# Plachtaa/FAcodec

Measured on AMD Instinct MI355X. Metric: 24kHz audio sec encoded+decoded per wall-sec, higher is better.
Workload: dtype f32; 1 GPU; configs[1]: batch=32/GPU x 2 s @ 24 kHz, forward encoder->FVQ(6 codebooks)->decoder, FAcodec configs/config.yml model (137.7 M params), weights formula-generated, weight-norm re-materialised every step; clips_per_gpu=32, samples_per_clip=48000, parallelism=dp1 (independent clips, no collective)

## Files before the change

facodec_amd/csrc/conv1d_bsplit.hip:

```cpp
#include "conv1d_mfma.h"
#include <type_traits>
#include "inflight_regs.h"
#include "prep_batch.h"

namespace fac {

typedef __bf16 bf16x8 __attribute__((ext_vector_type(8)));

constexpr int BS_CO = 64;
constexpr int BS_NSW = 4;
constexpr int BS_NSW_WIDE = 4;
constexpr int BS_XU = 3;
static int conv_device_cus() {
  static int cus[16] = {0};
  int dev = 0, v = 0;
  if (hipGetDevice(&dev) != hipSuccess || dev < 0 || dev >= 16) return 0;
  if (cus[dev] == 0 && hipDeviceGetAttribute(&v, hipDeviceAttributeMultiprocessorCount, dev) == hipSuccess) cus[dev] = v;
  return cus[dev];
}
constexpr int BS_WIDE_MIN = 64;
__host__ __device__ constexpr int bs_group(int C_in) { return C_in >= BS_WIDE_MIN ? 2 : 1; }

__device__ __forceinline__ void split3(float x, __bf16& h, __bf16& m, __bf16& l) {
  h = (__bf16)x;
  const float r1 = x - (float)h;
  m = (__bf16)r1;
  l = (__bf16)(r1 - (float)m);
}

__host__ __device__ constexpr int bs_slots(int K, int G) { return (G * K + 1) & ~1; }

__device__ __forceinline__ void pack_conv_split_body(const float* __restrict__ v, const float* __restrict__ scale,
                                                     bf16x8* __restrict__ out, int C_out, int C_in, int K, int G, int H, int n_st,
                                                     long long n, int vb, int vg) {
  for (long long idx = (long long)vb * 256 + threadIdx.x; idx < n; idx += (long long)vg * 256) {
    const int co = (int)(idx % BS_CO);
    long long r = idx / BS_CO;
    const int hs = (int)(r % H);
    r /= H;
    const int s = (int)(r % n_st);
    const int ct = (int)(r / n_st);
    const int g = hs % G, k = hs / G;
    const int cog = ct * BS_CO + co;
    const float sc = (scale != nullptr && cog < C_out) ? scale[cog] : 1.0f;
    bf16x8 h, m, l;
#pragma unroll
    for (int i = 0; i < 8; ++i) {
      const int ci = (s * G + g) * 8 + i;
      float w = 0.f;
      if (cog < C_out && ci < C_in && k < K) {
        w = v[((long long)cog * C_in + ci) * K + k];
        if (scale != nullptr) w = __fmul_rn(w, sc);
      }
      __bf16 a, b2, c;
      split3(w, a, b2, c);
      h[i] = a; m[i] = b2; l[i] = c;
    }
    const long long base = ((long long)ct * n_st + s) * 3;
    out[((base + 0) * H + hs) * BS_CO + co] = h;
    out[((base + 1) * H + hs) * BS_CO + co] = m;
    out[((base + 2) * H + hs) * BS_CO + co] = l;
  }
}

__global__ __launch_bounds__(256) void pack_conv_split_kernel(const float* __restrict__ v, const float* __restrict__ scale,
                                                              bf16x8* __restrict__ out, int C_out, int C_in, int K, int G, int H,
                                                              int n_st, long long n) {
  pack_conv_split_body(v, scale, out, C_out, C_in, K, G, H, n_st, n, blockIdx.x, gridDim.x);
}

__global__ __launch_bounds__(256) void bsplit_batch_kernel(const PrepJob* __restrict__ jobs, const int* __restrict__ first, int njobs) {
  const int j = prep_find_job(first, njobs, blockIdx.x);
  const PrepJob& J = jobs[j];
  pack_conv_split_body(static_cast<const float*>(J.a), static_cast<const float*>(J.b), static_cast<bf16x8*>(J.out), J.i[0], J.i[1],
                       J.i[2], J.i[3], J.i[4], J.i[5], J.n, blockIdx.x - first[j], J.nblocks);
}

int prep_launch_bsplit(const PrepJob* jobs, const int* first, int njobs, int total, hipStream_t s) {
  hipLaunchKernelGGL(bsplit_batch_kernel, dim3(total), dim3(256), 0, s, jobs, first, njobs);
  return check_launch("bsplit_batch");
}

template <int KT, int G, int NMW, int NSW>
__global__ __launch_bounds__((NMW + NSW) * 64, (NMW + NSW) / 4) void conv1d_bsplit_kernel(ConvArgs a) {
  constexpr int MB = 2, NB = 2;
  constexpr int BS_TT = 64 * NMW;
  constexpr int H = bs_slots(KT, G);
  constexpr int W_STAGE = 3 * H * BS_CO * 16;
  extern __shared__ __attribute__((aligned(16))) unsigned char sm[];
  const int tid = threadIdx.x;
  const int lane = tid & 63;
  const int wave = __builtin_amdgcn_readfirstlane(tid >> 6);
  const int XW = a.XW;
  const int X_STAGE = 48 * G * XW;
  const int STG = W_STAGE + X_STAGE;
  unsigned char* Wbuf = sm;
  unsigned char* Xbuf = sm + W_STAGE;
  const int n_chunks = (a.C_in + 8 * G - 1) / (8 * G);
  const int dil = a.dil;

  const int n_tiles = a.n_tiles;
  typedef const __attribute__((address_space(4))) ConvArgs* KArgP;
  const KArgP kargs = (KArgP)__builtin_amdgcn_kernarg_segment_ptr();
  auto fresh_args = [&]() {
    KArgP q = kargs;
    asm volatile("" : "+s"(q));
    return q;
  };
  auto decode = [&](KArgP ka, int v, int& t0_, int& co0_, int& b_) {
    const int q8 = n_tiles >> 3, r8 = n_tiles & 7;
    const int xcd = v & 7, within = v >> 3;
    const int id = (xcd < r8 ? xcd * (q8 + 1) : r8 * (q8 + 1) + (xcd - r8) * q8) + within;
    const int nt = ka->n_t_tiles;
    const int tt = id % nt;
    const int rest = id / nt;
    const int nb = ka->B;
    b_ = rest % nb;
    co0_ = (rest / nb) * BS_CO;
    t0_ = tt * BS_TT;
  };
  const bool overlap = a.persist != 0;
  unsigned char* epi_base = sm + (overlap ? STG : 0);
  auto walk = [&](auto role) {
  constexpr int ROLE = decltype(role)::value;
  constexpr bool STAGING = ROLE != 0;
  bool first = true;
  unsigned cboff[BS_XU] = {}, nboff[BS_XU] = {};
  unsigned long long cmask[BS_XU] = {}, nmask[BS_XU] = {};
  const float *cxg = nullptr, *nxg = nullptr;
  const unsigned char *cws = nullptr, *nws = nullptr;
  for (int vb = blockIdx.x; vb < n_tiles; vb += gridDim.x) {
  int t0, co0, b;
  decode(fresh_args(), vb, t0, co0, b);
  const bool has_nt = overlap && vb + (int)gridDim.x < n_tiles;

  if constexpr (STAGING) {
    const int lw = wave - NMW;
    __builtin_amdgcn_s_setprio(FAC_PRIO_STAGE);
    const float* xg = a.x + (long long)b * a.x_bs;
    const int xcs = (int)a.x_cs;
    const unsigned char* wsrc = reinterpret_cast<const unsigned char*>(a.w) + (long long)(co0 / BS_CO) * n_chunks * W_STAGE;
    const int n_blk = (XW + 63) >> 6;
    int u_g[BS_XU], u_c[BS_XU], u_idx[BS_XU];
#pragma unroll
    for (int j = 0; j < BS_XU; ++j) {
      const int u = lw + NSW * j;
      u_g[j] = u % G;
      const int c = (u / G) * 64 + lane;
      u_c[j] = (u < G * n_blk && c < XW) ? c : -1;
      const int tin = t0 - a.pad_left + c;
      int idx;
      if (a.pad_mode == FAC_PAD_REFLECT) idx = reflect_index(tin, a.T_in, a.T_ext);
      else idx = (tin >= 0 && tin < a.T_in) ? tin : -1;
      u_idx[j] = u_c[j] >= 0 ? idx : -1;
    }
    constexpr int NBLK = W_STAGE / 1024;
    constexpr int ND = (NBLK + NSW - 1) / NSW;
    constexpr int NX = BS_XU * 8;
    static_assert(W_STAGE % 1024 == 0 && ND + NX <= 63 && NX == 24, "vmcnt is a 6-bit counter; FAC_XREGS24_* list 24 registers per set");
    auto stage_w = [&](int chunk, int buf) {
      constexpr int N16 = W_STAGE / 16;
      const unsigned char* src = wsrc + (long long)chunk * W_STAGE;
      unsigned char* dst = Wbuf + buf * STG;
      for (int i = lw; i * 64 < N16; i += NSW) {
        const int q = i * 64 + lane;
        if (q < N16)
          __builtin_amdgcn_global_load_lds((glb_void_t*)(src + (long long)q * 16), (lds_void_t*)(dst + i * 1024), 16, 0, 0);
      }
    };
    auto write_x = [&](int buf, const float (&xr)[BS_XU][8]) {
      unsigned char* xd = Xbuf + buf * STG;
#pragma unroll
      for (int j = 0; j < BS_XU; ++j) {
        if (u_c[j] < 0) continue;
        bf16x8 h, m, l;
#pragma unroll
        for (int i = 0; i < 8; ++i) {
          __bf16 p0, p1, p2;
          split3(xr[j][i], p0, p1, p2);
          h[i] = p0; m[i] = p1; l[i] = p2;
        }
        *reinterpret_cast<bf16x8*>(xd + ((0 * G + u_g[j]) * XW + u_c[j]) * 16) = h;
        *reinterpret_cast<bf16x8*>(xd + ((1 * G + u_g[j]) * XW + u_c[j]) * 16) = m;
        *reinterpret_cast<bf16x8*>(xd + ((2 * G + u_g[j]) * XW + u_c[j]) * 16) = l;
      }
    };
    if constexpr (ROLE == 2) {
      typedef float wv4 __attribute__((ext_vector_type(4)));
      const unsigned char* xp = a.x_p8 + (long long)b * (a.C_in / 8) * a.T_in * 16;
      const long long grp_bytes = (long long)a.T_in * 16;
      unsigned u_poff[BS_XU];
      bool any_pad = false;
#pragma unroll
      for (int j = 0; j < BS_XU; ++j) {
        u_poff[j] = (unsigned)(u_idx[j] >= 0 ? u_idx[j] : 0) * 16u;
        any_pad = any_pad || __builtin_amdgcn_ballot_w64(u_c[j] >= 0 && u_idx[j] < 0) != 0;
      }
      for (int c = -1; c < n_chunks; ++c) {
        if (c + 1 < n_chunks) {
          const int buf = (c + 1) & 1;
          wv4 wv[ND], xv[BS_XU][3];
          const unsigned char* src = wsrc + (long long)(c + 1) * W_STAGE;
#pragma unroll
          for (int j = 0; j < ND; ++j) {
            const int bi = min(lw + NSW * j, NBLK - 1);
            wv[j] = *reinterpret_cast<const wv4*>(src + bi * 1024 + lane * 16);
          }
#pragma unroll
          for (int j = 0; j < BS_XU; ++j) {
            const unsigned char* grp = xp + (long long)((c + 1) * G + u_g[j]) * grp_bytes;
#pragma unroll
            for (int pl = 0; pl < 3; ++pl) xv[j][pl] = *reinterpret_cast<const wv4*>(grp + pl * a.x_p8_ps + u_poff[j]);
          }
          unsigned char* xd = Xbuf + buf * STG;
#pragma unroll
          for (int j = 0; j < BS_XU; ++j) {
            if (u_c[j] < 0) continue;
#pragma unroll
            for (int pl = 0; pl < 3; ++pl) {
              wv4 v = xv[j][pl];
              if (any_pad && u_idx[j] < 0) v = wv4{0.f, 0.f, 0.f, 0.f};
              *reinterpret_cast<wv4*>(xd + ((pl * G + u_g[j]) * XW + u_c[j]) * 16) = v;
            }
          }
          unsigned char* dst = Wbuf + buf * STG;
#pragma unroll
          for (int j = 0; j < ND; ++j) {
            const int bi = min(lw + NSW * j, NBLK - 1);
            *reinterpret_cast<wv4*>(dst + bi * 1024 + lane * 16) = wv[j];
          }
        }
        __syncthreads();
      }
    } else if constexpr (G == 2) {
#define BS_LD(n, R)                                                                                                          \
  asm volatile("global_load_dword v" #R ", %0, %1" : : "v"(u_boff[(n) / 8]), "s"(grp[(n) / 8] + (long long)((n) % 8) * xcs) : "memory", "v" #R);
#define BS_RD(n, R) asm volatile("v_cndmask_b32_e64 %0, 0, v" #R ", %1" : "=v"(xr[(n) / 8][(n) % 8]) : "s"(u_mask[(n) / 8]) : "memory");
      auto tile_params = [&](int t0_, int b_, int co0_, unsigned (&boff)[BS_XU], unsigned long long (&mask)[BS_XU], const float*& xgp,
                             const unsigned char*& wsp) {
        const KArgP ka = fresh_args();
        const int pad_left = ka->pad_left, pad_mode = ka->pad_mode, T_in = ka->T_in, T_ext = ka->T_ext;
#pragma unroll
        for (int j = 0; j < BS_XU; ++j) {
          const int tin = t0_ - pad_left + u_c[j];
          int idx;
          if (pad_mode == FAC_PAD_REFLECT) idx = reflect_index(tin, T_in, T_ext);
          else idx = (tin >= 0 && tin < T_in) ? tin : -1;
          if (u_c[j] < 0) idx = -1;
          boff[j] = (unsigned)(idx >= 0 ? idx : 0) * 4u;
          mask[j] = __builtin_amdgcn_ballot_w64(idx >= 0);
        }
        xgp = ka->x + (long long)b_ * ka->x_bs;
        wsp = reinterpret_cast<const unsigned char*>(ka->w) + (long long)(co0_ / BS_CO) * n_chunks * W_STAGE;
      };
      if (first) tile_params(t0, b, co0, cboff, cmask, cxg, cws);
      if (has_nt) {
        int nt0, nco0, nb;
        decode(fresh_args(), vb + (int)gridDim.x, nt0, nco0, nb);
        tile_params(nt0, nb, nco0, nboff, nmask, nxg, nws);
      }
      auto load_a = [&](const float* xgp, const unsigned (&u_boff)[BS_XU], int chunk) {
        const float* grp[BS_XU];
#pragma unroll
        for (int j = 0; j < BS_XU; ++j) grp[j] = xgp + (long long)((chunk * G + u_g[j]) * 8) * xcs;
        FAC_XREGS24_A(BS_LD)
      };
      auto load_b = [&](const float* xgp, const unsigned (&u_boff)[BS_XU], int chunk) {
        const float* grp[BS_XU];
#pragma unroll
        for (int j = 0; j < BS_XU; ++j) grp[j] = xgp + (long long)((chunk * G + u_g[j]) * 8) * xcs;
        FAC_XREGS24_B(BS_LD)
      };
      auto take_a = [&](float (&xr)[BS_XU][8], const unsigned long long (&u_mask)[BS_XU]) { FAC_XREGS24_A(BS_RD) };
      auto take_b = [&](float (&xr)[BS_XU][8], const unsigned long long (&u_mask)[BS_XU]) { FAC_XREGS24_B(BS_RD) };
      typedef float wv4 __attribute__((ext_vector_type(4)));
      const int wblk0 = min(lw * ND, NBLK - ND);
      const unsigned lane16 = (unsigned)lane * 16u;
      for (int base = first ? -2 : 0; base < n_chunks; base += 2) {
#pragma unroll
        for (int i = 0; i < 2; ++i) {
          const int c = base + i;
          if (c >= n_chunks) break;
          const bool nx1 = c + 1 >= n_chunks, nx2 = c + 2 >= n_chunks;
          const bool has_next = c + 1 >= 0 && (!nx1 || has_nt), has_next2 = !nx2 || has_nt;
          float xr[BS_XU][8];
          wv4 wv[ND];
          if (has_next) {
            const unsigned char* src = (nx1 ? nws : cws) + (long long)(nx1 ? c + 1 - n_chunks : c + 1) * W_STAGE + wblk0 * 1024;
#pragma unroll
            for (int j = 0; j < ND; ++j)
              asm volatile("global_load_dwordx4 %0, %1, %2" : "=v"(wv[j]) : "v"(lane16), "s"(src + j * 1024) : "memory");
            asm volatile("s_waitcnt vmcnt(%0)" : : "n"(ND) : "memory");
            unsigned long long u_mask[BS_XU];
#pragma unroll
            for (int j = 0; j < BS_XU; ++j) u_mask[j] = nx1 ? nmask[j] : cmask[j];
            if (i == 0) take_b(xr, u_mask); else take_a(xr, u_mask);
          }
          if (has_next2) {
            unsigned u_boff[BS_XU];
#pragma unroll
            for (int j = 0; j < BS_XU; ++j) u_boff[j] = nx2 ? nboff[j] : cboff[j];
            const float* xgp = nx2 ? nxg : cxg;
            const int chunk = nx2 ? c + 2 - n_chunks : c + 2;
            if (i == 0) load_a(xgp, u_boff, chunk); else load_b(xgp, u_boff, chunk);
          }
          if (has_next) {
            write_x(1 - i, xr);
            if (has_next2) asm volatile("s_waitcnt vmcnt(%0)" : : "n"(NX) : "memory");
            else asm volatile("s_waitcnt vmcnt(0)" ::: "memory");
            unsigned char* dst = Wbuf + (1 - i) * STG + wblk0 * 1024 + lane16;
#pragma unroll
            for (int j = 0; j < ND; ++j) {
              asm volatile("" : "+v"(wv[j]) : : "memory");
              *reinterpret_cast<wv4*>(dst + j * 1024) = wv[j];
            }
          }
          if (c >= -1) {
            asm volatile("s_waitcnt lgkmcnt(0)" ::: "memory");
            __builtin_amdgcn_s_barrier();
            asm volatile("" ::: "memory");
          }
        }
      }
      if (has_nt) {
#pragma unroll
        for (int j = 0; j < BS_XU; ++j) {
          cboff[j] = nboff[j];
          cmask[j] = nmask[j];
        }
        cxg = nxg;
        cws = nws;
      }
#undef BS_LD
#undef BS_RD
    } else {
      int u_off[BS_XU];
#pragma unroll
      for (int j = 0; j < BS_XU; ++j) u_off[j] = u_idx[j] >= 0 ? u_idx[j] : 0;
      auto load_x = [&](int chunk, float (&xr)[BS_XU][8]) {
#pragma unroll
        for (int j = 0; j < BS_XU; ++j) {
          const float* grp = xg + (long long)((chunk * G + u_g[j]) * 8) * xcs;
#pragma unroll
          for (int i = 0; i < 8; ++i) {
            const float v = (grp + (long long)i * xcs)[u_off[j]];
            xr[j][i] = u_idx[j] >= 0 ? v : 0.f;
          }
        }
      };
      float xa[BS_XU][8], xb[BS_XU][8];
      load_x(0, xa);
      stage_w(0, 0);
      if (n_chunks > 1) load_x(1, xb);
      write_x(0, xa);
      __syncthreads();
      for (int chunk = 0; chunk < n_chunks; chunk += 2) {
        if (chunk + 1 < n_chunks) {
          stage_w(chunk + 1, 1);
          if (chunk + 2 < n_chunks) load_x(chunk + 2, xa);
          write_x(1, xb);
        }
        __syncthreads();
        if (chunk + 1 >= n_chunks) break;
        if (chunk + 2 < n_chunks) {
          stage_w(chunk + 2, 0);
          if (chunk + 3 < n_chunks) load_x(chunk + 3, xb);
          write_x(0, xa);
        }
        __syncthreads();
      }
    }
    __builtin_amdgcn_s_setprio(0);
  } else {
  __builtin_amdgcn_s_setprio(FAC_PRIO_MFMA);
  const int l31 = lane & 31;
  const int kq = lane >> 5;
  const int n0 = wave * 64;
  f32x16 acc[MB][NB];
#pragma unroll
  for (int m = 0; m < MB; ++m)
#pragma unroll
    for (int n = 0; n < NB; ++n)
#pragma unroll
      for (int r = 0; r < 16; ++r) acc[m][n][r] = 0.f;

  const int x_lane = (G == 2 ? kq * XW : kq * dil) * 16;
  const int x_step = (G == 2 ? dil : 2 * dil) * 16;

  if (first) __syncthreads();
  if constexpr (NMW == 4) {
    constexpr int S = H / 2;
    auto pipeline = [&](auto MBc) {
    constexpr int MBv = decltype(MBc)::value;
    bf16x8 A[2][MBv][3], Bf[2][NB][3];
    auto ld = [&](int buf, int st, bf16x8 (&Ad)[MBv][3], bf16x8 (&Bd)[NB][3]) {
      const unsigned char* Wb = Wbuf + buf * STG + (kq * BS_CO + l31) * 16;
      const unsigned char* Xb = Xbuf + buf * STG + (n0 + l31) * 16 + x_lane + st * x_step;
      constexpr int PO[3] = {1, 0, 2};
#pragma unroll
      for (int pi = 0; pi < 3; ++pi) {
#pragma unroll
        for (int n = 0; n < NB; ++n) Bd[n][PO[pi]] = *reinterpret_cast<const bf16x8*>(Xb + (PO[pi] * G * XW + n * 32) * 16);
#pragma unroll
        for (int m = 0; m < MBv; ++m) Ad[m][PO[pi]] = *reinterpret_cast<const bf16x8*>(Wb + ((PO[pi] * H + 2 * st) * BS_CO + m * 32) * 16);
      }
    };
    auto mma = [&](const bf16x8 (&Ac)[MBv][3], const bf16x8 (&Bc)[NB][3]) {
      constexpr int TA[6] = {1, 2, 0, 1, 0, 0}, TB[6] = {1, 0, 2, 0, 1, 0};
#pragma unroll
      for (int q = 0; q < 6; ++q)
#pragma unroll
        for (int m = 0; m < MBv; ++m)
#pragma unroll
          for (int n = 0; n < NB; ++n) acc[m][n] = __builtin_amdgcn_mfma_f32_32x32x16_bf16(Ac[m][TA[q]], Bc[n][TB[q]], acc[m][n], 0, 0, 0);
    };
    auto interleave = [&]() {
#pragma unroll
      for (int i = 0; i < 3 * (MBv + NB); ++i) {
        __builtin_amdgcn_sched_group_barrier(0x008, (6 * MBv * NB) / (3 * (MBv + NB)) > 0 ? (6 * MBv * NB) / (3 * (MBv + NB)) : 1, 0);
        __builtin_amdgcn_sched_group_barrier(0x100, 1, 0);
      }
    };
    ld(0, 0, A[0], Bf[0]);
    for (int base = 0; base < n_chunks; base += 2) {
#pragma unroll
      for (int cc = 0; cc < 2; ++cc) {
        const int chunk = base + cc;
        if (chunk >= n_chunks) break;
        const int buf = cc;
#pragma unroll
        for (int st = 0; st < S; ++st) {
          const int cur = (cc * S + st) & 1;
          if (st + 1 < S) {
            if (cur == 0) ld(buf, st + 1, A[1], Bf[1]); else ld(buf, st + 1, A[0], Bf[0]);
            if (cur == 0) mma(A[0], Bf[0]); else mma(A[1], Bf[1]);
            interleave();
            __builtin_amdgcn_sched_barrier(0);
          } else {
            asm volatile("s_waitcnt lgkmcnt(0)" ::: "memory");
            __builtin_amdgcn_s_barrier();
            asm volatile("" ::: "memory");
            __builtin_amdgcn_sched_barrier(0);
            if (chunk + 1 < n_chunks) {
              if (cur == 0) ld(buf ^ 1, 0, A[1], Bf[1]); else ld(buf ^ 1, 0, A[0], Bf[0]);
            }
            if (cur == 0) mma(A[0], Bf[0]); else mma(A[1], Bf[1]);
            if (chunk + 1 < n_chunks) interleave();
            __builtin_amdgcn_sched_barrier(0);
          }
        }
      }
    }
    };
    if (co0 + 32 >= a.C_out) pipeline(std::integral_constant<int, 1>{});
    else pipeline(std::integral_constant<int, MB>{});
  } else {
  for (int chunk = 0; chunk < n_chunks; ++chunk) {
    const int buf = chunk & 1;
    const unsigned char* Wb = Wbuf + buf * STG + (kq * BS_CO + l31) * 16;
    const unsigned char* Xb = Xbuf + buf * STG + (n0 + l31) * 16 + x_lane;
    bf16x8 A[2][MB][3], Bf[1][NB][3];
    auto ldA = [&](int st, bf16x8 (&Ad)[MB][3]) {
#pragma unroll
      for (int p = 0; p < 3; ++p)
#pragma unroll
        for (int m = 0; m < MB; ++m)
          Ad[m][p] = *reinterpret_cast<const bf16x8*>(Wb + ((p * H + 2 * st) * BS_CO + m * 32) * 16);
    };
    auto ldB = [&](int st, bf16x8 (&Bd)[NB][3]) {
      const int xo = st * x_step;
      constexpr int PO[3] = {1, 0, 2};
#pragma unroll
      for (int pi = 0; pi < 3; ++pi)
#pragma unroll
        for (int n = 0; n < NB; ++n)
          Bd[n][PO[pi]] = *reinterpret_cast<const bf16x8*>(Xb + xo + (PO[pi] * G * XW + n * 32) * 16);
    };
#pragma unroll
    for (int st = 0; st < H / 2; ++st) {
      ldB(st, Bf[0]);
      ldA(st, A[0]);
      __builtin_amdgcn_sched_barrier(0);
      constexpr int TA[6] = {1, 2, 0, 1, 0, 0}, TB[6] = {1, 0, 2, 0, 1, 0};
#pragma unroll
      for (int q = 0; q < 6; ++q)
#pragma unroll
        for (int m = 0; m < MB; ++m)
#pragma unroll
          for (int n = 0; n < NB; ++n)
            acc[m][n] = __builtin_amdgcn_mfma_f32_32x32x16_bf16(A[0][m][TA[q]], Bf[0][n][TB[q]], acc[m][n], 0, 0, 0);
      __builtin_amdgcn_sched_barrier(0);
    }
    __syncthreads();
  }
  }
  __builtin_amdgcn_s_setprio(0);
  {
    float* tile = reinterpret_cast<float*>(epi_base);
    constexpr int EP = BS_TT + 4;
#pragma unroll
    for (int m = 0; m < MB; ++m)
#pragma unroll
      for (int n = 0; n < NB; ++n)
#pragma unroll
        for (int r = 0; r < 16; ++r)
          tile[(m * 32 + (r & 3) + 8 * (r >> 2) + 4 * kq) * EP + n0 + n * 32 + l31] = acc[m][n][r];
  }
  }
  __syncthreads();

  {
    const KArgP e = fresh_args();
    const float* tile = reinterpret_cast<const float*>(epi_base);
    constexpr int EP = BS_TT + 4;
    constexpr int NTH = (NMW + NSW) * 64;
    constexpr int QPR = BS_TT / 4;
    float* yg = e->y ? e->y + (long long)b * e->y_bs : nullptr;
    float* y2g = e->y2 ? e->y2 + (long long)b * e->y_bs : nullptr;
    const float* rg = e->res ? e->res + (long long)b * e->y_bs : nullptr;
    const bool vec_ok = (e->y_cs & 3) == 0 && (e->y_bs & 3) == 0 && (!yg || (reinterpret_cast<unsigned long long>(e->y) & 15) == 0) &&
                        (!y2g || (reinterpret_cast<unsigned long long>(e->y2) & 15) == 0) &&
                        (!rg || (reinterpret_cast<unsigned long long>(e->res) & 15) == 0);
    for (int q = tid; q < BS_CO * QPR; q += NTH) {
      const int row = q / QPR, tq = q - row * QPR;
      const int co = co0 + row, t = t0 + 4 * tq;
      if (co >= e->C_out || t >= e->T_out) continue;
      const float4 av = *reinterpret_cast<const float4*>(tile + row * EP + 4 * tq);
      float v[4] = {av.x, av.y, av.z, av.w};
      const float bs = e->bias ? e->bias[co] : 0.f;
      const float al = e->alpha_out ? e->alpha_out[co] : 0.f;
      const float inv = e->alpha_out ? snake_inv(al) : 0.f;
      const long long o = (long long)co * e->y_cs + t;
      const bool full = vec_ok && t + 3 < e->T_out;
      float rv[4] = {0.f, 0.f, 0.f, 0.f};
      if (rg) {
        if (full) {
          const float4 r4 = *reinterpret_cast<const float4*>(rg + o);
          rv[0] = r4.x; rv[1] = r4.y; rv[2] = r4.z; rv[3] = r4.w;
        } else {
#pragma unroll
          for (int i = 0; i < 4; ++i) rv[i] = t + i < e->T_out ? rg[o + i] : 0.f;
        }
      }
#pragma unroll
      for (int i = 0; i < 4; ++i) {
        float x = v[i] + bs;
        if (e->alpha_out) x = snake_apply(x, al, inv);
        if (e->act != FAC_ACT_NONE) x = apply_act_slow(x, e->act);
        v[i] = x + rv[i];
      }
      float w[4];
      if (y2g) {
        const float a2 = e->alpha2[co], i2 = snake_inv(a2);
#pragma unroll
        for (int i = 0; i < 4; ++i) w[i] = snake_apply(v[i], a2, i2);
      }
      if (full) {
        if (yg) *reinterpret_cast<float4*>(yg + o) = make_float4(v[0], v[1], v[2], v[3]);
        if (y2g) *reinterpret_cast<float4*>(y2g + o) = make_float4(w[0], w[1], w[2], w[3]);
      } else {
#pragma unroll
        for (int i = 0; i < 4; ++i) {
          if (t + i >= e->T_out) continue;
          if (yg) yg[o + i] = v[i];
          if (y2g) y2g[o + i] = w[i];
        }
      }
    }
  }
  first = !overlap;
  if (vb + (int)gridDim.x < n_tiles) __syncthreads();
  }
  };
  if (wave >= NMW) {
    if constexpr (G == 2) {
      if (a.x_p8 != nullptr) walk(std::integral_constant<int, 2>{});
      else walk(std::integral_constant<int, 1>{});
    } else {
      walk(std::integral_constant<int, 1>{});
    }
  } else {
    walk(std::integral_constant<int, 0>{});
  }
}

bool conv_bsplit_ok(const ConvArgs& a) {
  if (!((a.K == 7 || a.K == 5 || a.K == 3) && a.stride == 1 && a.n_phase == 1 && a.phase_shift == 0 && a.y_tstride == 1 && !a.alpha_in &&
        !a.w1 && !a.w_batched && (long long)a.B * a.T_out > 640))
    return false;
  const int G = bs_group(a.C_in), tt = G == 2 ? 256 : 512;
  const int kp = G == 2 ? a.K - 1 : ((a.K + 1) & ~1) - 1;
  return a.C_in % (8 * G) == 0 && G * ((tt + kp * a.dil + 63) / 64) <= BS_NSW * BS_XU &&
         a.x_cs * (long long)a.C_in < (1ll << 31);
}

bool conv_bsplit_p8_ok(const ConvArgs& a) {
  return conv_bsplit_ok(a) && bs_group(a.C_in) == 2 && (long long)a.T_in * 16 < (1ll << 32);
}

template <int KT, int G, int NMW, int NSW>
static int bsplit_launch(ConvArgs& a, hipStream_t s) {
  constexpr int H = bs_slots(KT, G), TT = 64 * NMW;
  a.XW = TT + (H / G - 1) * a.dil;
  const size_t stg = (size_t)3 * H * BS_CO * 16 + (size_t)48 * G * a.XW;
  const size_t epi = (size_t)BS_CO * (TT + 4) * sizeof(float);
  a.n_t_tiles = (a.T_out + TT - 1) / TT;
  const long long n_wg = (long long)a.n_t_tiles * ((a.C_out + BS_CO - 1) / BS_CO) * a.B;
  if (n_wg > 0x7fffffffll) {
    set_error("conv1d: too many workgroups (%lld)", n_wg);
    return FAC_ERR_ARG;
  }
  const int n_chunks = (a.C_in + 8 * G - 1) / (8 * G);
  int cus = conv_device_cus() & ~7;
  a.persist = (G == 2 && NMW == 4 && a.x_p8 == nullptr && n_chunks % 2 == 0 && cus >= 8 && n_wg > cus &&
               stg + (stg > epi ? stg : epi) <= 160 * 1024) ? 1 : 0;
  size_t lds = a.persist ? stg + (stg > epi ? stg : epi) : (2 * stg > epi ? 2 * stg : epi);
  if (lds > 160 * 1024) {
    set_error("conv1d(bf16 split): tile needs %zu B of LDS (dil=%d)", lds, a.dil);
    return FAC_ERR_ARG;
  }
  auto kern = conv1d_bsplit_kernel<KT, G, NMW, NSW>;
  static bool attr_set = false;
  if (!attr_set) {
    (void)hipFuncSetAttribute(reinterpret_cast<const void*>(kern), hipFuncAttributeMaxDynamicSharedMemorySize, 160 * 1024);
    attr_set = true;
  }
  a.n_tiles = (int)n_wg;
  hipLaunchKernelGGL(kern, dim3((unsigned)(a.persist ? cus : n_wg)), dim3((NMW + NSW) * 64), lds, s, a);
  return check_launch("conv1d_bsplit");
}

int conv_dispatch_bsplit(ConvArgs& a, hipStream_t s) {
  if (a.K == 5)
    return bs_group(a.C_in) == 2 ? bsplit_launch<5, 2, 4, BS_NSW_WIDE>(a, s) : bsplit_launch<5, 1, 8, BS_NSW>(a, s);
  if (a.K == 3)
    return bs_group(a.C_in) == 2 ? bsplit_launch<3, 2, 4, BS_NSW_WIDE>(a, s) : bsplit_launch<3, 1, 8, BS_NSW>(a, s);
  return bs_group(a.C_in) == 2 ? bsplit_launch<7, 2, 4, BS_NSW_WIDE>(a, s) : bsplit_launch<7, 1, 8, BS_NSW>(a, s);
}

}

extern "C" int fac_debug_bsplit_occupancy(int lds_bytes) {
  int n = -1;
  auto kern = fac::conv1d_bsplit_kernel<7, 2, 4, fac::BS_NSW_WIDE>;
  (void)hipFuncSetAttribute(reinterpret_cast<const void*>(kern), hipFuncAttributeMaxDynamicSharedMemorySize, 160 * 1024);
  if (hipOccupancyMaxActiveBlocksPerMultiprocessor(&n, kern, (4 + fac::BS_NSW) * 64, (size_t)lds_bytes) != hipSuccess) return -1;
  return n;
}

extern "C" int64_t fac_conv_w_split_bytes(int C_out, int C_in, int K) {
  using namespace fac;
  const int G = bs_group(C_in);
  const int64_t n_ct = (C_out + BS_CO - 1) / BS_CO, n_st = (C_in + 8 * G - 1) / (8 * G);
  return n_ct * n_st * 3 * bs_slots(K, G) * BS_CO * 16;
}

extern "C" int fac_pack_conv_w_split(const float* v, const float* scale, void* out, int C_out, int C_in, int K,
                                     fac_stream_t stream) {
  using namespace fac;
  FAC_REQUIRE(v && out && C_out > 0 && C_in > 0 && K > 0, "pack_conv_w_split: bad arguments");
  const int G = bs_group(C_in);
  const int n_ct = (C_out + BS_CO - 1) / BS_CO, n_st = (C_in + 8 * G - 1) / (8 * G), H = bs_slots(K, G);
  const long long n = (long long)n_ct * n_st * H * BS_CO;
  const int blocks = (int)((n + 255) / 256 < 65535 ? (n + 255) / 256 : 65535);
  if (prep_recording()) {
    PrepJob j{}; j.a = v; j.b = scale; j.out = out; j.kind = PK_CONV_SPLIT; j.nblocks = blocks; j.n = n;
    j.i[0] = C_out; j.i[1] = C_in; j.i[2] = K; j.i[3] = G; j.i[4] = H; j.i[5] = n_st;
    return prep_record(PU_BSPLIT, j);
  }
  hipLaunchKernelGGL(pack_conv_split_kernel, dim3(blocks), dim3(256), 0, (hipStream_t)stream, v, scale,
                     reinterpret_cast<bf16x8*>(out), C_out, C_in, K, G, H, n_st, n);
  return check_launch("pack_conv_w_split");
}
```

Before: 1206 audio-s/s.

## Stream conv weights from global via buffer loads instead of staging in LDS

For the wide-channel NMW=4 path, compute waves now read weight fragments directly from global memory with raw buffer loads held in a register ring that runs two steps ahead, instead of having staging waves copy weights into LDS. This takes the weight staging traffic and the LDS footprint for weights out of the pipeline, and the epilogue gets its own LDS region. The cost is more global/L2 load pressure from the compute waves, higher register use for the A ring, and reliance on cache hits for weights shared across tiles.

```diff
diff --git a/facodec_amd/csrc/conv1d_bsplit.hip b/facodec_amd/csrc/conv1d_bsplit.hip
--- a/facodec_amd/csrc/conv1d_bsplit.hip
+++ b/facodec_amd/csrc/conv1d_bsplit.hip
@@ -11,6 +11,7 @@
 constexpr int BS_NSW = 4;
 constexpr int BS_NSW_WIDE = 4;
 constexpr int BS_XU = 3;
+constexpr int BS_WAHEAD = 2;
 static int conv_device_cus() {
   static int cus[16] = {0};
   int dev = 0, v = 0;
@@ -87,15 +88,17 @@
   constexpr int BS_TT = 64 * NMW;
   constexpr int H = bs_slots(KT, G);
   constexpr int W_STAGE = 3 * H * BS_CO * 16;
+  constexpr bool WSTREAM = NMW == 4 && G == 2;
+  constexpr int W_LDS = WSTREAM ? 0 : W_STAGE;
   extern __shared__ __attribute__((aligned(16))) unsigned char sm[];
   const int tid = threadIdx.x;
   const int lane = tid & 63;
   const int wave = __builtin_amdgcn_readfirstlane(tid >> 6);
   const int XW = a.XW;
   const int X_STAGE = 48 * G * XW;
-  const int STG = W_STAGE + X_STAGE;
+  const int STG = W_LDS + X_STAGE;
   unsigned char* Wbuf = sm;
-  unsigned char* Xbuf = sm + W_STAGE;
+  unsigned char* Xbuf = sm + W_LDS;
   const int n_chunks = (a.C_in + 8 * G - 1) / (8 * G);
   const int dil = a.dil;
 
@@ -120,7 +123,7 @@
     t0_ = tt * BS_TT;
   };
   const bool overlap = a.persist != 0;
-  unsigned char* epi_base = sm + (overlap ? STG : 0);
+  unsigned char* epi_base = sm + (WSTREAM ? 2 * STG : 0);
   auto walk = [&](auto role) {
   constexpr int ROLE = decltype(role)::value;
   constexpr bool STAGING = ROLE != 0;
@@ -128,7 +131,6 @@
   unsigned cboff[BS_XU] = {}, nboff[BS_XU] = {};
   unsigned long long cmask[BS_XU] = {}, nmask[BS_XU] = {};
   const float *cxg = nullptr, *nxg = nullptr;
-  const unsigned char *cws = nullptr, *nws = nullptr;
   for (int vb = blockIdx.x; vb < n_tiles; vb += gridDim.x) {
   int t0, co0, b;
   decode(fresh_args(), vb, t0, co0, b);
@@ -154,11 +156,9 @@
       else idx = (tin >= 0 && tin < a.T_in) ? tin : -1;
       u_idx[j] = u_c[j] >= 0 ? idx : -1;
     }
-    constexpr int NBLK = W_STAGE / 1024;
-    constexpr int ND = (NBLK + NSW - 1) / NSW;
     constexpr int NX = BS_XU * 8;
-    static_assert(W_STAGE % 1024 == 0 && ND + NX <= 63 && NX == 24, "vmcnt is a 6-bit counter; FAC_XREGS24_* list 24 registers per set");
-    auto stage_w = [&](int chunk, int buf) {
+    static_assert(W_STAGE % 1024 == 0 && NX == 24, "FAC_XREGS24_* list 24 registers per set");
+    [[maybe_unused]] auto stage_w = [&](int chunk, int buf) {
       constexpr int N16 = W_STAGE / 16;
       const unsigned char* src = wsrc + (long long)chunk * W_STAGE;
       unsigned char* dst = Wbuf + buf * STG;
@@ -199,13 +199,7 @@
       for (int c = -1; c < n_chunks; ++c) {
         if (c + 1 < n_chunks) {
           const int buf = (c + 1) & 1;
-          wv4 wv[ND], xv[BS_XU][3];
-          const unsigned char* src = wsrc + (long long)(c + 1) * W_STAGE;
-#pragma unroll
-          for (int j = 0; j < ND; ++j) {
-            const int bi = min(lw + NSW * j, NBLK - 1);
-            wv[j] = *reinterpret_cast<const wv4*>(src + bi * 1024 + lane * 16);
-          }
+          wv4 xv[BS_XU][3];
 #pragma unroll
           for (int j = 0; j < BS_XU; ++j) {
             const unsigned char* grp = xp + (long long)((c + 1) * G + u_g[j]) * grp_bytes;
@@ -223,12 +217,6 @@
               *reinterpret_cast<wv4*>(xd + ((pl * G + u_g[j]) * XW + u_c[j]) * 16) = v;
             }
           }
-          unsigned char* dst = Wbuf + buf * STG;
-#pragma unroll
-          for (int j = 0; j < ND; ++j) {
-            const int bi = min(lw + NSW * j, NBLK - 1);
-            *reinterpret_cast<wv4*>(dst + bi * 1024 + lane * 16) = wv[j];
-          }
         }
         __syncthreads();
       }
@@ -236,8 +224,7 @@
 #define BS_LD(n, R)                                                                                                          \
   asm volatile("global_load_dword v" #R ", %0, %1" : : "v"(u_boff[(n) / 8]), "s"(grp[(n) / 8] + (long long)((n) % 8) * xcs) : "memory", "v" #R);
 #define BS_RD(n, R) asm volatile("v_cndmask_b32_e64 %0, 0, v" #R ", %1" : "=v"(xr[(n) / 8][(n) % 8]) : "s"(u_mask[(n) / 8]) : "memory");
-      auto tile_params = [&](int t0_, int b_, int co0_, unsigned (&boff)[BS_XU], unsigned long long (&mask)[BS_XU], const float*& xgp,
-                             const unsigned char*& wsp) {
+      auto tile_params = [&](int t0_, int b_, unsigned (&boff)[BS_XU], unsigned long long (&mask)[BS_XU], const float*& xgp) {
         const KArgP ka = fresh_args();
         const int pad_left = ka->pad_left, pad_mode = ka->pad_mode, T_in = ka->T_in, T_ext = ka->T_ext;
 #pragma unroll
@@ -251,13 +238,12 @@
           mask[j] = __builtin_amdgcn_ballot_w64(idx >= 0);
         }
         xgp = ka->x + (long long)b_ * ka->x_bs;
-        wsp = reinterpret_cast<const unsigned char*>(ka->w) + (long long)(co0_ / BS_CO) * n_chunks * W_STAGE;
       };
-      if (first) tile_params(t0, b, co0, cboff, cmask, cxg, cws);
+      if (first) tile_params(t0, b, cboff, cmask, cxg);
       if (has_nt) {
         int nt0, nco0, nb;
         decode(fresh_args(), vb + (int)gridDim.x, nt0, nco0, nb);
-        tile_params(nt0, nb, nco0, nboff, nmask, nxg, nws);
+        tile_params(nt0, nb, nboff, nmask, nxg);
       }
       auto load_a = [&](const float* xgp, const unsigned (&u_boff)[BS_XU], int chunk) {
         const float* grp[BS_XU];
@@ -273,9 +259,6 @@
       };
       auto take_a = [&](float (&xr)[BS_XU][8], const unsigned long long (&u_mask)[BS_XU]) { FAC_XREGS24_A(BS_RD) };
       auto take_b = [&](float (&xr)[BS_XU][8], const unsigned long long (&u_mask)[BS_XU]) { FAC_XREGS24_B(BS_RD) };
-      typedef float wv4 __attribute__((ext_vector_type(4)));
-      const int wblk0 = min(lw * ND, NBLK - ND);
-      const unsigned lane16 = (unsigned)lane * 16u;
       for (int base = first ? -2 : 0; base < n_chunks; base += 2) {
 #pragma unroll
         for (int i = 0; i < 2; ++i) {
@@ -284,13 +267,8 @@
           const bool nx1 = c + 1 >= n_chunks, nx2 = c + 2 >= n_chunks;
           const bool has_next = c + 1 >= 0 && (!nx1 || has_nt), has_next2 = !nx2 || has_nt;
           float xr[BS_XU][8];
-          wv4 wv[ND];
           if (has_next) {
-            const unsigned char* src = (nx1 ? nws : cws) + (long long)(nx1 ? c + 1 - n_chunks : c + 1) * W_STAGE + wblk0 * 1024;
-#pragma unroll
-            for (int j = 0; j < ND; ++j)
-              asm volatile("global_load_dwordx4 %0, %1, %2" : "=v"(wv[j]) : "v"(lane16), "s"(src + j * 1024) : "memory");
-            asm volatile("s_waitcnt vmcnt(%0)" : : "n"(ND) : "memory");
+            asm volatile("s_waitcnt vmcnt(0)" ::: "memory");
             unsigned long long u_mask[BS_XU];
 #pragma unroll
             for (int j = 0; j < BS_XU; ++j) u_mask[j] = nx1 ? nmask[j] : cmask[j];
@@ -304,17 +282,7 @@
             const int chunk = nx2 ? c + 2 - n_chunks : c + 2;
             if (i == 0) load_a(xgp, u_boff, chunk); else load_b(xgp, u_boff, chunk);
           }
-          if (has_next) {
-            write_x(1 - i, xr);
-            if (has_next2) asm volatile("s_waitcnt vmcnt(%0)" : : "n"(NX) : "memory");
-            else asm volatile("s_waitcnt vmcnt(0)" ::: "memory");
-            unsigned char* dst = Wbuf + (1 - i) * STG + wblk0 * 1024 + lane16;
-#pragma unroll
-            for (int j = 0; j < ND; ++j) {
-              asm volatile("" : "+v"(wv[j]) : : "memory");
-              *reinterpret_cast<wv4*>(dst + j * 1024) = wv[j];
-            }
-          }
+          if (has_next) write_x(1 - i, xr);
           if (c >= -1) {
             asm volatile("s_waitcnt lgkmcnt(0)" ::: "memory");
             __builtin_amdgcn_s_barrier();
@@ -329,7 +297,6 @@
           cmask[j] = nmask[j];
         }
         cxg = nxg;
-        cws = nws;
       }
 #undef BS_LD
 #undef BS_RD
@@ -387,23 +354,35 @@
   const int x_lane = (G == 2 ? kq * XW : kq * dil) * 16;
   const int x_step = (G == 2 ? dil : 2 * dil) * 16;
 
-  if (first) __syncthreads();
   if constexpr (NMW == 4) {
     constexpr int S = H / 2;
+    constexpr int RING = BS_WAHEAD + 1;
+    constexpr int NCH = (2 * S) % RING == 0 ? 2 : 2 * RING;
+    typedef unsigned u32x4 __attribute__((ext_vector_type(4)));
+    const auto wrsrc = __builtin_amdgcn_make_buffer_rsrc(
+        const_cast<unsigned char*>(reinterpret_cast<const unsigned char*>(a.w)) + (long long)(co0 / BS_CO) * n_chunks * W_STAGE, 0,
+        n_chunks * W_STAGE, 0x00020000);
+    int w_off[3];
+#pragma unroll
+    for (int p = 0; p < 3; ++p) w_off[p] = ((p * H + kq) * BS_CO + l31) * 16;
     auto pipeline = [&](auto MBc) {
     constexpr int MBv = decltype(MBc)::value;
-    bf16x8 A[2][MBv][3], Bf[2][NB][3];
-    auto ld = [&](int buf, int st, bf16x8 (&Ad)[MBv][3], bf16x8 (&Bd)[NB][3]) {
-      const unsigned char* Wb = Wbuf + buf * STG + (kq * BS_CO + l31) * 16;
+    bf16x8 A[RING][MBv][3], Bf[2][NB][3];
+    constexpr int PO[3] = {1, 0, 2};
+    auto ldA = [&](int chunk, int st, bf16x8 (&Ad)[MBv][3]) {
+      const int so = min(chunk, n_chunks - 1) * W_STAGE + st * (2 * BS_CO * 16);
+#pragma unroll
+      for (int pi = 0; pi < 3; ++pi)
+#pragma unroll
+        for (int m = 0; m < MBv; ++m)
+          Ad[m][PO[pi]] = __builtin_bit_cast(bf16x8, __builtin_amdgcn_raw_buffer_load_b128(wrsrc, w_off[PO[pi]] + m * 512, so, 0));
+    };
+    auto ldB = [&](int buf, int st, bf16x8 (&Bd)[NB][3]) {
       const unsigned char* Xb = Xbuf + buf * STG + (n0 + l31) * 16 + x_lane + st * x_step;
-      constexpr int PO[3] = {1, 0, 2};
-#pragma unroll
-      for (int pi = 0; pi < 3; ++pi) {
+#pragma unroll
+      for (int pi = 0; pi < 3; ++pi)
 #pragma unroll
         for (int n = 0; n < NB; ++n) Bd[n][PO[pi]] = *reinterpret_cast<const bf16x8*>(Xb + (PO[pi] * G * XW + n * 32) * 16);
-#pragma unroll
-        for (int m = 0; m < MBv; ++m) Ad[m][PO[pi]] = *reinterpret_cast<const bf16x8*>(Wb + ((PO[pi] * H + 2 * st) * BS_CO + m * 32) * 16);
-      }
     };
     auto mma = [&](const bf16x8 (&Ac)[MBv][3], const bf16x8 (&Bc)[NB][3]) {
       constexpr int TA[6] = {1, 2, 0, 1, 0, 0}, TB[6] = {1, 0, 2, 0, 1, 0};
@@ -415,25 +394,33 @@
           for (int n = 0; n < NB; ++n) acc[m][n] = __builtin_amdgcn_mfma_f32_32x32x16_bf16(Ac[m][TA[q]], Bc[n][TB[q]], acc[m][n], 0, 0, 0);
     };
     auto interleave = [&]() {
-#pragma unroll
-      for (int i = 0; i < 3 * (MBv + NB); ++i) {
-        __builtin_amdgcn_sched_group_barrier(0x008, (6 * MBv * NB) / (3 * (MBv + NB)) > 0 ? (6 * MBv * NB) / (3 * (MBv + NB)) : 1, 0);
-        __builtin_amdgcn_sched_group_barrier(0x100, 1, 0);
-      }
-    };
-    ld(0, 0, A[0], Bf[0]);
-    for (int base = 0; base < n_chunks; base += 2) {
-#pragma unroll
-      for (int cc = 0; cc < 2; ++cc) {
+      constexpr int NM = 6 * MBv * NB, NR = 3 * (MBv + NB);
+      constexpr int PER = NM / NR > 0 ? NM / NR : 1;
+#pragma unroll
+      for (int i = 0; i < NR; ++i) {
+        __builtin_amdgcn_sched_group_barrier(0x008, PER, 0);
+        if (i % 2 == 0 && i / 2 < 3 * MBv) __builtin_amdgcn_sched_group_barrier(0x020, 1, 0);
+        else __builtin_amdgcn_sched_group_barrier(0x100, 1, 0);
+      }
+    };
+#pragma unroll
+    for (int j = 0; j < BS_WAHEAD; ++j) ldA(j / S, j % S, A[j % RING]);
+    if (first) __syncthreads();
+    ldB(0, 0, Bf[0]);
+    for (int base = 0; base < n_chunks; base += NCH) {
+#pragma unroll
+      for (int cc = 0; cc < NCH; ++cc) {
         const int chunk = base + cc;
         if (chunk >= n_chunks) break;
-        const int buf = cc;
+        const int buf = cc & 1;
 #pragma unroll
         for (int st = 0; st < S; ++st) {
-          const int cur = (cc * S + st) & 1;
+          const int j = cc * S + st;
+          const int ja = j + BS_WAHEAD;
           if (st + 1 < S) {
-            if (cur == 0) ld(buf, st + 1, A[1], Bf[1]); else ld(buf, st + 1, A[0], Bf[0]);
-            if (cur == 0) mma(A[0], Bf[0]); else mma(A[1], Bf[1]);
+            ldA(base + ja / S, ja % S, A[ja % RING]);
+            ldB(buf, st + 1, Bf[(j + 1) & 1]);
+            mma(A[j % RING], Bf[j & 1]);
             interleave();
             __builtin_amdgcn_sched_barrier(0);
           } else {
@@ -441,11 +428,10 @@
             __builtin_amdgcn_s_barrier();
             asm volatile("" ::: "memory");
             __builtin_amdgcn_sched_barrier(0);
-            if (chunk + 1 < n_chunks) {
-              if (cur == 0) ld(buf ^ 1, 0, A[1], Bf[1]); else ld(buf ^ 1, 0, A[0], Bf[0]);
-            }
-            if (cur == 0) mma(A[0], Bf[0]); else mma(A[1], Bf[1]);
-            if (chunk + 1 < n_chunks) interleave();
+            ldA(base + ja / S, ja % S, A[ja % RING]);
+            ldB(buf ^ 1, 0, Bf[(j + 1) & 1]);
+            mma(A[j % RING], Bf[j & 1]);
+            interleave();
             __builtin_amdgcn_sched_barrier(0);
           }
         }
@@ -455,6 +441,7 @@
     if (co0 + 32 >= a.C_out) pipeline(std::integral_constant<int, 1>{});
     else pipeline(std::integral_constant<int, MB>{});
   } else {
+  if (first) __syncthreads();
   for (int chunk = 0; chunk < n_chunks; ++chunk) {
     const int buf = chunk & 1;
     const unsigned char* Wb = Wbuf + buf * STG + (kq * BS_CO + l31) * 16;
@@ -602,7 +589,8 @@
 static int bsplit_launch(ConvArgs& a, hipStream_t s) {
   constexpr int H = bs_slots(KT, G), TT = 64 * NMW;
   a.XW = TT + (H / G - 1) * a.dil;
-  const size_t stg = (size_t)3 * H * BS_CO * 16 + (size_t)48 * G * a.XW;
+  constexpr bool WSTREAM = NMW == 4 && G == 2;
+  const size_t stg = (WSTREAM ? 0 : (size_t)3 * H * BS_CO * 16) + (size_t)48 * G * a.XW;
   const size_t epi = (size_t)BS_CO * (TT + 4) * sizeof(float);
   a.n_t_tiles = (a.T_out + TT - 1) / TT;
   const long long n_wg = (long long)a.n_t_tiles * ((a.C_out + BS_CO - 1) / BS_CO) * a.B;
@@ -612,9 +600,8 @@
   }
   const int n_chunks = (a.C_in + 8 * G - 1) / (8 * G);
   int cus = conv_device_cus() & ~7;
-  a.persist = (G == 2 && NMW == 4 && a.x_p8 == nullptr && n_chunks % 2 == 0 && cus >= 8 && n_wg > cus &&
-               stg + (stg > epi ? stg : epi) <= 160 * 1024) ? 1 : 0;
-  size_t lds = a.persist ? stg + (stg > epi ? stg : epi) : (2 * stg > epi ? 2 * stg : epi);
+  a.persist = (WSTREAM && a.x_p8 == nullptr && n_chunks % 2 == 0 && cus >= 8 && n_wg > cus) ? 1 : 0;
+  size_t lds = WSTREAM ? 2 * stg + epi : (2 * stg > epi ? 2 * stg : epi);
   if (lds > 160 * 1024) {
     set_error("conv1d(bf16 split): tile needs %zu B of LDS (dil=%d)", lds, a.dil);
     return FAC_ERR_ARG;
```

Result: no change. 1217 audio-s/s (median of 6 runs) (+1.0%).
